# fraunhoferhhi/vvdec

Hardware: NVIDIA H100
Metric: decoded frames/sec, 4K 10-bit Main10 RA, bit-exact YUV vs reference (higher is better)
Workload: dtype int16 samples / int32 accumulate

## Files before the change

vvdec_b200/csrc/k2_inter.cu:

```cuda
#define VVC_TABLE_QUAL static __device__ const __align__(16)
#include "vvc_tables.h"
#include "common.cuh"
#include <algorithm>
#include <cuda.h>

namespace b200 {

constexpr int IFO = 8192;

struct McParams {
  int16_t* dst[3]; int dstStride[3];
  const int16_t* refs[B200_MAX_SLOTS * 3];
  int refStride[3];
  int W, H, bitDepth, ctuSize, chroma;
  int fastOk;
  const b200_pu* pus; const uint32_t* tiles; const int* meta;
  int32_t* dmvrMv;
  const b200_wp* wp;
  const b200_lmcs* lmcs; int lmcsLog2;
  const CUtensorMap* tmaps; uint8_t tmapBuf[B200_MAX_SLOTS];
};

constexpr int TMA_LW = 24, TMA_LH = 23, TMA_CW = 16, TMA_CH = 11;
constexpr int TMA_LWIN = 576, TMA_CWIN = 192;
__device__ __forceinline__ unsigned smem_u32(const void* p) { return (unsigned)__cvta_generic_to_shared(p); }
__device__ __forceinline__ void mbar_init(unsigned long long* bar, int count)
{
  asm volatile("mbarrier.init.shared::cta.b64 [%0], %1;" :: "r"(smem_u32(bar)), "r"(count) : "memory");
  asm volatile("fence.mbarrier_init.release.cluster;" ::: "memory");
}
__device__ __forceinline__ void mbar_expect_tx(unsigned long long* bar, int bytes)
{
  asm volatile("mbarrier.arrive.expect_tx.release.cta.shared::cta.b64 _, [%0], %1;" :: "r"(smem_u32(bar)), "r"(bytes) : "memory");
}
__device__ __forceinline__ void mbar_wait(unsigned long long* bar, int parity)
{
  asm volatile("{\n\t.reg .pred P1;\n\tWAIT_%=:\n\tmbarrier.try_wait.parity.shared::cta.b64 P1, [%0], %1;\n\t@P1 bra DONE_%=;\n\tbra WAIT_%=;\n\tDONE_%=:\n\t}"
               :: "r"(smem_u32(bar)), "r"(parity) : "memory");
}
__device__ __forceinline__ void tma_load_2d(void* smemDst, const CUtensorMap* map, int x, int y, unsigned long long* bar)
{
  asm volatile("cp.async.bulk.tensor.2d.shared::cluster.global.tile.mbarrier::complete_tx::bytes [%0], [%1, {%2, %3}], [%4];"
               :: "r"(smem_u32(smemDst)), "l"(map), "r"(x), "r"(y), "r"(smem_u32(bar)) : "memory");
}

__device__ __forceinline__ void cp_async4(void* smemDst, const void* gmemSrc)
{
  const unsigned d = (unsigned)__cvta_generic_to_shared(smemDst);
  asm volatile("cp.async.ca.shared.global [%0], [%1], 4;\n" :: "r"(d), "l"(gmemSrc));
}
__device__ __forceinline__ void cp_async_wait_all() { asm volatile("cp.async.wait_all;\n" ::: "memory"); }

#define LUMA_OUT(v) (P.lmcs ? lmcs_fwd(P.lmcs, P.lmcsLog2, (v), pmax) : (v))

struct RefPl { const int16_t* p; int w, h, stride; };
__device__ __forceinline__ int ldc(const RefPl& r, int x, int y) { return r.p[(size_t)min(max(y, 0), r.h - 1) * r.stride + min(max(x, 0), r.w - 1)]; }
struct Win { int x0, y0, x1, y1; };
__device__ __forceinline__ int ldw(const RefPl& r, const Win& W, int x, int y) { return ldc(r, min(max(x, W.x0), W.x1), min(max(y, W.y0), W.y1)); }

__device__ __forceinline__ void clip_mv(int& mx, int& my, int x, int y, const McParams& P)
{
  mx = clip3((-P.ctuSize - 8 - x + 1) * 16, (P.W + 8 - x - 1) * 16, mx);
  my = clip3((-P.ctuSize - 8 - y + 1) * 16, (P.H + 8 - y - 1) * 16, my);
}

__device__ __forceinline__ const int8_t* luma_taps(int frac, bool is4x4, bool altHpel)
{
  if (is4x4) return kIfLuma4x4 + frac * 8;
  if (frac == 8 && altHpel) return kIfAltHpel;
  return kIfLuma + frac * 8;
}

__device__ __forceinline__ void load_taps8(const int8_t* t, int f[8])
{
  const int2 w = __ldg(reinterpret_cast<const int2*>(t));
#pragma unroll
  for (int k = 0; k < 4; k++) { f[k] = (w.x << (24 - 8 * k)) >> 24; f[4 + k] = (w.y << (24 - 8 * k)) >> 24; }
}

__device__ __forceinline__ int avg_bi(int p0, int p1, int w1, int hr, int pmax)
{
  int v;
  if (w1 == 4) v = (p0 + p1 + (1 << hr) + 2 * IFO) >> (hr + 1);
  else         v = (p0 * (8 - w1) + p1 * w1 + (1 << (hr + 2)) + (IFO << 3)) >> (hr + 3);
  return clip3(0, pmax, v);
}

__device__ __forceinline__ int wp_uni(const b200_wp* e, int comp, int p, int hr, int pmax)
{
  const int s = e->shift[comp] + hr;
  return clip3(0, pmax, ((e->w0[comp] * (p + IFO) + (s > 0 ? 1 << (s - 1) : 0)) >> s) + e->offset[comp]);
}
__device__ __forceinline__ int wp_bi(const b200_wp* e, int comp, int p0, int p1, int hr, int pmax)
{
  const int s = e->shift[comp] + hr;
  return clip3(0, pmax, (e->w0[comp] * (p0 + IFO) + e->w1[comp] * (p1 + IFO) + ((1 << s) >> 1) + e->offset[comp] * (1 << (s - 1))) >> s);
}

__device__ __forceinline__ int geo_weight(int splitDir, int l2w, int l2h, int x, int y, int sc)
{
  const int angle = kGeoParams[splitDir * 2], mir = kGeoAngle2Mirror[angle];
  const int16_t* wo = &kGeoWeightOffset[((splitDir * 4 + (l2h - 3)) * 4 + (l2w - 3)) * 2];
  const int row = mir == 2 ? VVC_GEO_MASK_SIZE - 1 - wo[1] - (y << sc) : wo[1] + (y << sc);
  const int col = mir == 1 ? VVC_GEO_MASK_SIZE - 1 - wo[0] - (x << sc) : wo[0] + (x << sc);
  return kGeoWeights[(kGeoAngle2Mask[angle] * VVC_GEO_MASK_SIZE + row) * VVC_GEO_MASK_SIZE + col];
}
__device__ __forceinline__ int geo_blend(int wt, int p0, int p1, int hr, int pmax)
{
  const int s = hr + 3;
  return clip3(0, pmax, (wt * p0 + (8 - wt) * p1 + (1 << (s - 1)) + (IFO << 3)) >> s);
}

__device__ __forceinline__ int shift_msb(int numer, int denom) { return numer >> (31 - __clz(denom)); }

__device__ int div_for_maxq7(long long N, long long D)
{
  int sign = 0, q = 0;
  if (N < 0) { sign = 1; N = -N; }
  D <<= 3;
  if (N >= D) { N -= D; q++; }
  q <<= 1; D >>= 1;
  if (N >= D) { N -= D; q++; }
  q <<= 1;
  if (N >= (D >> 1)) q++;
  return sign ? -q : q;
}

struct TileSmem {
  int16_t *w[2], *h[2];
  int16_t *cw[2][2], *chf[2][2];
  int16_t *p[2];
};

constexpr int HS = 16, CHS = 8;
constexpr int DMVR_TAIL = 1640;

__host__ __device__ inline int mc_smem_elems(int mode, int n, bool tma = false)
{
  if (tma) {
    const int lists = mode == 0 ? 1 : 2;
    int e = lists * (TMA_LWIN + 23 * HS + 2 * (TMA_CWIN + 11 * CHS));
    if (mode >= 2) e = max(e, 8 * n) + 2 * 324;
    return (e + 64 + 64) & ~7;
  }
  const int win = n == 256 ? 552 : n == 128 ? 368 : n == 64 ? 276 : 180;
  const int hf  = (n == 256 ? 23 : n == 128 ? 23 : n == 64 ? 23 : 15) * HS;
  const int cwin = n == 256 ? 132 : n == 128 ? 88 : n == 64 ? 66 : 42;
  const int chf = (n == 256 ? 11 : n == 128 ? 11 : n == 64 ? 11 : 7) * CHS;
  const int lists = mode == 0 ? 1 : 2;
  int e = lists * (win + hf + 2 * (cwin + chf));
  if (mode == 3) e = max(e, 2 * 441);
  if (mode >= 2) e = max(e, 8 * n);
  if (mode == 3) e += DMVR_TAIL;
  if (mode >= 2) e += 2 * 324;
  return (e + 64) & ~7;
}

template <int MODE, int OPT, bool TMA>
__device__ __forceinline__ void mc_tile(const McParams& P, const uint32_t tile, int16_t* smem, unsigned* sSad, int* sDec, int (*sVxy)[2], unsigned long long* sBar)
{
  const int tid = threadIdx.x, nthr = blockDim.x;
  const b200_pu& pu = P.pus[tile >> 6];
  const int puW = pu.w, puH = pu.h, puX = pu.x, puY = pu.y, flags = pu.flags;
  const int tx0 = (tile & 7) * 16, ty0 = ((tile >> 3) & 7) * 16;
  const int tw = min(16, puW - tx0), th = min(16, puH - ty0);
  const int l2w = 31 - __clz(tw);
  const int bx = puX + tx0, by = puY + ty0;
  const int bd = P.bitDepth, pmax = (1 << bd) - 1, hr = max(2, 14 - bd), sh1 = 6 - hr;
  constexpr bool BI = MODE != 0;
  const bool altHpel = flags & B200_PU_ALTHPEL;
  const bool is4x4 = puW == 4 && puH == 4;
  const int l0 = BI ? 0 : (pu.refSlot[0] >= 0 ? 0 : 1);
  constexpr int NL = BI ? 2 : 1;
  const int cw = tw >> 1, ch = th >> 1, l2cw = l2w - 1;
  const int chroma = P.chroma;
  const b200_wp* we = (MODE <= 1 && P.wp && pu.wpIdx) ? P.wp + pu.wpIdx - 1 : nullptr;
  const bool geo = MODE == 1 && (flags & B200_PU_GEO);
  const int gl2w = 31 - __clz(puW), gl2h = 31 - __clz(puH);
  const int WS = tw + 8, CS = TMA ? TMA_CW : cw + 4;

  TileSmem S;
  int16_t* tail = smem;
  {
    int16_t* q = smem;
    const int win = WS * (th + 7), hf = (th + 7) * HS, cwin = CS * (ch + 3), chf = (ch + 3) * CHS;
    if (TMA) {
      q += ((128 - (smem_u32(smem) & 127)) & 127) >> 1;
#pragma unroll
      for (int l = 0; l < NL; l++) { S.w[l] = q; q += TMA_LWIN; }
#pragma unroll
      for (int l = 0; l < NL; l++)
#pragma unroll
        for (int c = 0; c < 2; c++) { S.cw[l][c] = q; q += TMA_CWIN; }
#pragma unroll
      for (int l = 0; l < NL; l++) { S.h[l] = q; q += hf; }
#pragma unroll
      for (int l = 0; l < NL; l++)
#pragma unroll
        for (int c = 0; c < 2; c++) { S.chf[l][c] = q; q += chf; }
    } else {
#pragma unroll
    for (int l = 0; l < NL; l++) { S.w[l] = q; q += win; S.h[l] = q; q += hf; }
#pragma unroll
    for (int l = 0; l < NL; l++)
#pragma unroll
      for (int c = 0; c < 2; c++) { S.cw[l][c] = q; q += cwin; S.chf[l][c] = q; q += chf; }
    }
    if (MODE == 3 && q < smem + 2 * 441) q = smem + 2 * 441;
    if (MODE >= 2) { if (q < smem + 8 * tw * th) q = smem + 8 * tw * th; if (MODE == 3) { tail = q; q += DMVR_TAIL; } S.p[0] = q; S.p[1] = q + 324; }
  }

  const int16_t* rp[NL][3]; int mvx[NL], mvy[NL]; int tbuf[NL];
#pragma unroll
  for (int li = 0; li < NL; li++) {
    const int l = BI ? li : l0;
    const int slot = pu.refSlot[l];
    if (TMA) tbuf[li] = P.tmapBuf[slot];
#pragma unroll
    for (int c = 0; c < 3; c++) rp[li][c] = P.refs[slot * 3 + c];
    mvx[li] = pu.mv[l][0]; mvy[li] = pu.mv[l][1];
  }
  const int W = P.W, H = P.H, CWp = W >> 1, CHp = H >> 1, rs0 = P.refStride[0], rs1 = P.refStride[1];
  int ox[NL], oy[NL], ocx[NL], ocy[NL];
  int wx0[NL][2], wy0[NL][2], wx1[NL][2], wy1[NL][2];
  int fmx[NL], fmy[NL];
  bool bio = MODE == 2;

  int wofs[NL], cofs[NL];
  bool dmvrFast = false;
  if (MODE == 3) {
    int16_t* B0 = tail; int16_t* B1 = tail + 400;
    int16_t* B0s = tail + 800; int16_t* B1s = tail + 1200;
    const int BW = tw + 4, BH = th + 4;
    const int warp = tid >> 5, lane = tid & 31, nw = max(1, nthr >> 5);
    int ix[2], iy[2], icx[2], icy[2];
    dmvrFast = P.fastOk;
#pragma unroll
    for (int li = 0; li < 2; li++) {
      ix[li] = bx + (mvx[li] >> 4); iy[li] = by + (mvy[li] >> 4); icx[li] = (bx >> 1) + (mvx[li] >> 5); icy[li] = (by >> 1) + (mvy[li] >> 5);
      dmvrFast = dmvrFast && ix[li] >= 6 && ix[li] + tw + 8 < W && iy[li] >= 6 && iy[li] + th + 8 < H;
      dmvrFast = dmvrFast && (!chroma || (icx[li] >= 4 && icx[li] + cw + 5 < CWp && icy[li] >= 3 && icy[li] + ch + 4 < CHp));
    }
    const int16_t* braw[2]; int bstr;
    int bxF[2], byF[2];
    if (dmvrFast) {
#pragma unroll
      for (int li = 0; li < 2; li++) {
        bxF[li] = mvx[li] & 15; byF[li] = mvy[li] & 15;
        wofs[li] = (ix[li] - 3) & 1;
        {
          const int half = lane >> 4, wl = lane & 15, rw = rs0 >> 1;
          const uint32_t* src = reinterpret_cast<const uint32_t*>(rp[li][0] + (size_t)(iy[li] - 3) * rs0 + ((ix[li] - 3) & ~1)) + (size_t)(warp * 2 + half) * rw + wl;
          uint32_t* dst = reinterpret_cast<uint32_t*>(S.w[li]) + (warp * 2 + half) * (WS >> 1) + wl;
          if (wl < (WS >> 1))
#pragma unroll 4
            for (int y = warp * 2 + half; y < th + 7; y += nw * 2) { cp_async4(dst, src); src += (size_t)(nw * 2) * rw; dst += nw * 2 * (WS >> 1); }
        }
        cofs[li] = (icx[li] - 1) & 1;
        if (chroma) {
          const int sub = lane >> 3, wl = lane & 7, rwc = rs1 >> 1, npc = (ch + 6) >> 2;
          const size_t cbase = (size_t)(icy[li] - 1) * rs1 + ((icx[li] - 1) & ~1);
          for (int q = warp; q < 2 * npc; q += nw) {
// ... 178 lines not shown
      }
    }
#pragma unroll
    for (int li = 0; li < NL; li++) {
      const bool fast = lfast[li];
      wofs[li] = (fast && !TMA) ? ((ox[li] - 3) & 1) : 0;
      if (fast && TMA) {
      } else if (fast) {
        const int half = lane >> 4, wl = lane & 15, rw = rs0 >> 1;
        const uint32_t* src = reinterpret_cast<const uint32_t*>(rp[li][0] + (size_t)(oy[li] - 3) * rs0 + ((ox[li] - 3) & ~1)) + (size_t)(warp * 2 + half) * rw + wl;
        uint32_t* dst = reinterpret_cast<uint32_t*>(S.w[li]) + (warp * 2 + half) * (WS >> 1) + wl;
        if (wl < (WS >> 1))
#pragma unroll 4
          for (int y = warp * 2 + half; y < th + 7; y += nw * 2) { cp_async4(dst, src); src += (size_t)(nw * 2) * rw; dst += nw * 2 * (WS >> 1); }
      } else {
        const int xlo = MODE == 3 ? clip3(0, W - 1, wx0[li][0]) : 0, xhi = MODE == 3 ? clip3(0, W - 1, wx1[li][0]) : W - 1;
        const int ylo = MODE == 3 ? clip3(0, H - 1, wy0[li][0]) : 0, yhi = MODE == 3 ? clip3(0, H - 1, wy1[li][0]) : H - 1;
        const int xc = min(max(ox[li] - 3 + lane, xlo), xhi);
        if (lane < tw + 7)
#pragma unroll 4
          for (int y = warp; y < th + 7; y += nw) S.w[li][y * WS + lane] = __ldg(rp[li][0] + (size_t)min(max(oy[li] - 3 + y, ylo), yhi) * rs0 + xc);
      }
      cofs[li] = 0;
      if (chroma) {
        const bool cfast = cfastv[li];
        cofs[li] = (cfast && !TMA) ? ((ocx[li] - 1) & 1) : 0;
        if (cfast && TMA) {
        } else if (cfast) {
          const int sub = lane >> 3, wl = lane & 7, rwc = rs1 >> 1, npc = (ch + 6) >> 2;
          const size_t cbase = (size_t)(ocy[li] - 1) * rs1 + ((ocx[li] - 1) & ~1);
          for (int q = warp; q < 2 * npc; q += nw) {
            const int c = q >= npc, y = ((c ? q - npc : q) << 2) + sub;
            if (y < ch + 3 && wl < ((cw + 4) >> 1))
              cp_async4(reinterpret_cast<uint32_t*>(c ? S.cw[li][1] : S.cw[li][0]) + y * (CS >> 1) + wl, reinterpret_cast<const uint32_t*>((c ? rp[li][2] : rp[li][1]) + cbase) + (size_t)y * rwc + wl);
          }
        } else {
          const int c = lane >> 4, xl = lane & 15;
          const int xlo = MODE == 3 ? clip3(0, CWp - 1, wx0[li][1]) : 0, xhi = MODE == 3 ? clip3(0, CWp - 1, wx1[li][1]) : CWp - 1;
          const int ylo = MODE == 3 ? clip3(0, CHp - 1, wy0[li][1]) : 0, yhi = MODE == 3 ? clip3(0, CHp - 1, wy1[li][1]) : CHp - 1;
          const int xcc = min(max(ocx[li] - 1 + xl, xlo), xhi);
          const int16_t* rc = c ? rp[li][2] : rp[li][1];
          int16_t* dc = c ? S.cw[li][1] : S.cw[li][0];
          if (xl < cw + 3)
#pragma unroll 4
            for (int y = warp; y < ch + 3; y += nw) dc[y * CS + xl] = __ldg(rc + (size_t)min(max(ocy[li] - 1 + y, ylo), yhi) * rs1 + xcc);
        }
      }
    }
  }
  cp_async_wait_all();
  if (TMA && tmaAny) mbar_wait(sBar, 0);
  __syncthreads();

#pragma unroll
  for (int li = 0; li < NL; li++) {
    int f[8];
    load_taps8(luma_taps(fmx[li] & 15, is4x4, altHpel), f);
    const int16_t* sw = S.w[li] + wofs[li];
    if (OPT == 1) {
      for (int i = tid; i < (th + 7) << l2w; i += nthr) {
        const int y = i >> l2w, x = i & (tw - 1);
        const int16_t* s = sw + y * WS + x;
        int a = 0;
#pragma unroll
        for (int k = 0; k < 8; k++) a += f[k] * s[k];
        S.h[li][y * HS + x] = (int16_t)((a - (IFO << sh1)) >> sh1);
      }
    } else {
      const int l2g = l2w - 2;
      for (int i = tid; i < (th + 7) << l2g; i += nthr) {
        const int y = i >> l2g, x = (i & ((tw >> 2) - 1)) << 2;
        const int16_t* s = sw + y * WS + x;
        int v[11];
#pragma unroll
        for (int k = 0; k < 11; k++) v[k] = s[k];
        int16_t* o = S.h[li] + y * HS + x;
#pragma unroll
        for (int j = 0; j < 4; j++) {
          int a = 0;
#pragma unroll
          for (int k = 0; k < 8; k++) a += f[k] * v[j + k];
          o[j] = (int16_t)((a - (IFO << sh1)) >> sh1);
        }
      }
    }
    if (chroma) {
      const int8_t* t = kIfChroma + (fmx[li] & 31) * 4;
      const int c0 = t[0], c1 = t[1], c2 = t[2], c3 = t[3];
      for (int i = tid; i < 2 * ((ch + 3) << l2cw); i += nthr) {
        const int c = i >= ((ch + 3) << l2cw), j = c ? i - ((ch + 3) << l2cw) : i;
        const int y = j >> l2cw, x = j & (cw - 1);
        const int16_t* s = (c ? S.cw[li][1] : S.cw[li][0]) + cofs[li] + y * CS + x;
        (c ? S.chf[li][1] : S.chf[li][0])[y * CHS + x] = (int16_t)((c0 * s[0] + c1 * s[1] + c2 * s[2] + c3 * s[3] - (IFO << sh1)) >> sh1);
      }
    }
  }
  __syncthreads();

  const int sx = tid & (tw - 1), sy = (tid >> l2w) * OPT;
  {
    int pr[NL][OPT];
#pragma unroll
    for (int li = 0; li < NL; li++) {
      int f[8];
      load_taps8(luma_taps(fmy[li] & 15, is4x4, altHpel), f);
      const int16_t* s = S.h[li] + sy * HS + sx;
      int v[7 + OPT];
#pragma unroll
      for (int k = 0; k < 7 + OPT; k++) v[k] = s[k * HS];
#pragma unroll
      for (int j = 0; j < OPT; j++) {
        int a = 0;
#pragma unroll
        for (int k = 0; k < 8; k++) a += f[k] * v[j + k];
        pr[li][j] = a;
      }
    }
#pragma unroll
    for (int j = 0; j < OPT; j++) {
      int16_t* d = P.dst[0] + (size_t)(by + sy + j) * P.dstStride[0] + bx + sx;
      if (MODE == 1 && geo) *d = (int16_t)LUMA_OUT(geo_blend(geo_weight(pu.bcwW1, gl2w, gl2h, tx0 + sx, ty0 + sy + j, 0), (int16_t)(pr[0][j] >> 6), (int16_t)(pr[NL - 1][j] >> 6), hr, pmax));
      else if (MODE <= 1 && we) *d = (int16_t)LUMA_OUT(BI ? wp_bi(we, 0, (int16_t)(pr[0][j] >> 6), (int16_t)(pr[NL - 1][j] >> 6), hr, pmax) : wp_uni(we, 0, (int16_t)(pr[0][j] >> 6), hr, pmax));
      else if (!BI) *d = (int16_t)LUMA_OUT(clip3(0, pmax, (pr[0][j] + (1 << (5 + hr)) + (IFO << 6)) >> (6 + hr)));
      else if (!bio) *d = (int16_t)LUMA_OUT(avg_bi((int16_t)(pr[0][j] >> 6), (int16_t)(pr[NL - 1][j] >> 6), MODE == 1 ? pu.bcwW1 : 4, hr, pmax));
      else { S.p[0][(sy + j + 1) * 18 + sx + 1] = (int16_t)(pr[0][j] >> 6); S.p[1][(sy + j + 1) * 18 + sx + 1] = (int16_t)(pr[NL - 1][j] >> 6); }
    }
  }
  if (chroma) {
    for (int i = tid; i < 2 * (ch << l2cw); i += nthr) {
      const int c = i >= (ch << l2cw), j = c ? i - (ch << l2cw) : i;
      const int y = j >> l2cw, x = j & (cw - 1);
      int pr[NL];
#pragma unroll
      for (int li = 0; li < NL; li++) {
        const int8_t* t = kIfChroma + (fmy[li] & 31) * 4;
        const int16_t* s = (c ? S.chf[li][1] : S.chf[li][0]) + y * CHS + x;
        pr[li] = t[0] * s[0] + t[1] * s[CHS] + t[2] * s[2 * CHS] + t[3] * s[3 * CHS];
      }
      int16_t* d = (c ? P.dst[2] : P.dst[1]) + (size_t)((by >> 1) + y) * (c ? P.dstStride[2] : P.dstStride[1]) + (bx >> 1) + x;
      if (MODE == 1 && geo) *d = (int16_t)geo_blend(geo_weight(pu.bcwW1, gl2w, gl2h, (tx0 >> 1) + x, (ty0 >> 1) + y, 1), (int16_t)(pr[0] >> 6), (int16_t)(pr[NL - 1] >> 6), hr, pmax);
      else if (MODE <= 1 && we) *d = (int16_t)(BI ? wp_bi(we, 1 + c, (int16_t)(pr[0] >> 6), (int16_t)(pr[NL - 1] >> 6), hr, pmax) : wp_uni(we, 1 + c, (int16_t)(pr[0] >> 6), hr, pmax));
      else if (!BI) *d = (int16_t)clip3(0, pmax, (pr[0] + (1 << (5 + hr)) + (IFO << 6)) >> (6 + hr));
      else *d = (int16_t)avg_bi((int16_t)(pr[0] >> 6), (int16_t)(pr[NL - 1] >> 6), MODE == 1 ? pu.bcwW1 : 4, hr, pmax);
    }
  }

  if (MODE >= 2) {
    if (!bio) return;
    for (int i = tid; i < 4 * (tw + th + 2); i += nthr) {
      const int li = i >= 2 * (tw + th + 2), j = li ? i - 2 * (tw + th + 2) : i;
      int x, y;
      if (j < tw + 2) { x = j; y = 0; } else if (j < 2 * (tw + 2)) { x = j - (tw + 2); y = th + 1; }
      else if (j < 2 * (tw + 2) + th) { x = 0; y = j - 2 * (tw + 2) + 1; } else { x = tw + 1; y = j - 2 * (tw + 2) - th + 1; }
      const int mxl = li ? fmx[NL - 1] : fmx[0], myl = li ? fmy[NL - 1] : fmy[0];
      const int xo = (mxl & 15) < 8 ? 1 : 0, yo = (myl & 15) < 8 ? 1 : 0;
      const int16_t* wl = li ? S.w[NL - 1] + wofs[NL - 1] : S.w[0] + wofs[0];
      const int v = wl[(y - yo + 3) * WS + (x - xo + 3)];
      (li ? S.p[1] : S.p[0])[y * 18 + x] = (int16_t)((int16_t)(v << hr) - IFO);
    }
    __syncthreads();
    uint4* Q = reinterpret_cast<uint4*>(smem);
    int dgx[OPT], dgy[OPT], psum[OPT];
    {
      int q0[OPT + 2], q1[OPT + 2];
#pragma unroll
      for (int r = 0; r < OPT + 2; r++) { q0[r] = S.p[0][(sy + r) * 18 + sx + 1] >> 6; q1[r] = S.p[1][(sy + r) * 18 + sx + 1] >> 6; }
#pragma unroll
      for (int j = 0; j < OPT; j++) {
        const int i = (sy + j + 1) * 18 + sx + 1;
        const int p0 = S.p[0][i], p1 = S.p[1][i];
        const int g0x = (S.p[0][i + 1] >> 6) - (S.p[0][i - 1] >> 6), g1x = (S.p[1][i + 1] >> 6) - (S.p[1][i - 1] >> 6);
        const int g0y = q0[j + 2] - q0[j], g1y = q1[j + 2] - q1[j];
        const int tX = (g0x + g1x) >> 1, tY = (g0y + g1y) >> 1, dI = (p1 >> 4) - (p0 >> 4);
        uint4 rec;
        rec.x = (unsigned)abs(tX) | ((unsigned)abs(tY) << 16);
        rec.y = (unsigned)(tX < 0 ? -dI : (tX == 0 ? 0 : dI));
        rec.z = (unsigned)(tY < 0 ? -dI : (tY == 0 ? 0 : dI));
        rec.w = (unsigned)(tY < 0 ? -tX : (tY == 0 ? 0 : tX));
        Q[((sy + j) << l2w) + sx] = rec;
        dgx[j] = g0x - g1x; dgy[j] = g0y - g1y; psum[j] = p0 + p1;
      }
    }
    __syncthreads();
    const int nBlk = (tw >> 2) * (th >> 2), l2bw = l2w - 2;
    for (int it = tid; it < ((nBlk * 4 + 31) & ~31); it += nthr) {
      const int blk = it >> 2, part = it & 3;
      unsigned sA = 0; int sDX = 0, sDY = 0, sS = 0;
      if (blk < nBlk) {
        const int bxx = (blk & ((tw >> 2) - 1)) << 2, byy = (blk >> l2bw) << 2;
#pragma unroll
        for (int rr = 0; rr < 2; rr++) {
          const int yy = part + 4 * rr;
          if (yy < 6) {
            const uint4* row = Q + (min(max(byy + yy - 1, 0), th - 1) << l2w);
#pragma unroll
            for (int xx = 0; xx < 6; xx++) {
              const uint4 r = row[min(max(bxx + xx - 1, 0), tw - 1)];
              sA += r.x; sDX += (int)r.y; sDY += (int)r.z; sS += (int)r.w;
            }
          }
        }
      }
#pragma unroll
      for (int m = 1; m < 4; m <<= 1) {
        sA += __shfl_xor_sync(0xffffffffu, sA, m);
        sDX += __shfl_xor_sync(0xffffffffu, sDX, m); sDY += __shfl_xor_sync(0xffffffffu, sDY, m);
        sS  += __shfl_xor_sync(0xffffffffu, sS, m);
      }
      if (part == 0 && blk < nBlk) {
        const int sAX = sA & 0xffff, sAY = sA >> 16;
        int vx = sAX == 0 ? 0 : shift_msb(sDX * 4, sAX);
        vx = clip3(-15, 15, vx);
        const int mainG = sS >> 12, secG = sS & 4095;
        int tmp = vx * mainG;
        tmp = ((tmp * (1 << 12)) + vx * secG) >> 1;
        int vy = sAY == 0 ? 0 : shift_msb(sDY * 4 - tmp, sAY);
        vy = clip3(-15, 15, vy);
        sVxy[blk][0] = vx; sVxy[blk][1] = vy;
      }
    }
    __syncthreads();
#pragma unroll
    for (int j = 0; j < OPT; j++) {
      const int y = sy + j, blk = ((y >> 2) << l2bw) + (sx >> 2);
      const int b = sVxy[blk][0] * dgx[j] + sVxy[blk][1] * dgy[j];
      const int shiftNum = 15 - bd, offset = (1 << (shiftNum - 1)) + 2 * IFO;
      P.dst[0][(size_t)(by + y) * P.dstStride[0] + bx + sx] = (int16_t)LUMA_OUT(clip3(0, pmax, (int)(int16_t)((psum[j] + b + offset) >> shiftNum)));
    }
  }
}

template <int MODE, int OPT, bool TMA>
__global__ void __launch_bounds__(64, MODE >= 2 ? 12 : 16) mc_kernel(const McParams P, const int list)
{
  extern __shared__ __align__(128) int16_t smem[];
  __shared__ unsigned sSad[25];
  __shared__ int sDec[3];
  __shared__ int sVxy[16][2];
  __shared__ __align__(8) unsigned long long sBar;
  if ((int)blockIdx.x >= P.meta[LM_CNT + list]) return;
  if (TMA) { if (threadIdx.x == 0) mbar_init(&sBar, 1); __syncthreads(); }
  mc_tile<MODE, OPT, TMA>(P, P.tiles[P.meta[LM_OFF + list] + blockIdx.x], smem, sSad, sDec, sVxy, &sBar);
}

__device__ __forceinline__ void round_affine(int& x, int& y, int s) { const int o = 1 << (s - 1); x = (x + o - (x >= 0)) >> s; y = (y + o - (y >= 0)) >> s; }

__device__ bool spread_over_limit(int a, int b, int c, int d, int predType)
{
  const int s4 = 4 << 11, ft = 6;
  if (predType == 3) {
    int rw = max(max(0, 4 * a + s4), max(4 * c, 4 * a + 4 * c + s4)) - min(min(0, 4 * a + s4), min(4 * c, 4 * a + 4 * c + s4));
    int rh = max(max(0, 4 * b), max(4 * d + s4, 4 * b + 4 * d + s4)) - min(min(0, 4 * b), min(4 * d + s4, 4 * b + 4 * d + s4));
    rw = (rw >> 11) + ft + 3; rh = (rh >> 11) + ft + 3;
    return rw * rh > (ft + 9) * (ft + 9);
  }
  int rw = max(0, 4 * a + s4) - min(0, 4 * a + s4), rh = max(0, 4 * b) - min(0, 4 * b);
  rw = (rw >> 11) + ft + 3; rh = (rh >> 11) + ft + 3;
  if (rw * rh > (ft + 9) * (ft + 5)) return true;
  rw = max(0, 4 * c) - min(0, 4 * c); rh = max(0, 4 * d + s4) - min(0, 4 * d + s4);
  rw = (rw >> 11) + ft + 3; rh = (rh >> 11) + ft + 3;
  return rw * rh > (ft + 5) * (ft + 9);
}

struct AffModel { int LTx, LTy, dHX, dHY, dVX, dVY; bool over, prof; };

__device__ void aff_model(const b200_pu& pu, int l, AffModel& M)
{
  const int l2w = 31 - __clz((int)pu.w), l2h = 31 - __clz((int)pu.h);
  M.LTx = pu.mv[l][0]; M.LTy = pu.mv[l][1];
  const int RTx = pu.cpmv[l][0][0], RTy = pu.cpmv[l][0][1], LBx = pu.cpmv[l][1][0], LBy = pu.cpmv[l][1][1];
  const bool six = pu.flags & B200_PU_AFFINE6;
  M.dHX = (RTx - M.LTx) * (1 << (7 - l2w)); M.dHY = (RTy - M.LTy) * (1 << (7 - l2w));
  M.dVX = six ? (LBx - M.LTx) * (1 << (7 - l2h)) : -M.dHY; M.dVY = six ? (LBy - M.LTy) * (1 << (7 - l2h)) : M.dHX;
  M.over = spread_over_limit(M.dHX, M.dHY, M.dVX, M.dVY, pu.interDir);
  bool prof = pu.flags & (l ? B200_PU_PROF1 : B200_PU_PROF0);
  if (six ? (M.LTx == RTx && M.LTy == RTy && M.LTx == LBx && M.LTy == LBy) : (M.LTx == RTx && M.LTy == RTy)) prof = false;
  if (M.over) prof = false;
  M.prof = prof;
}

__device__ __forceinline__ void aff_sub_mv(const AffModel& M, const b200_pu& pu, int i, int j, int& mx, int& my)
{
  if (M.over) { mx = M.LTx * 128 + M.dHX * (pu.w >> 1) + M.dVX * (pu.h >> 1); my = M.LTy * 128 + M.dHY * (pu.w >> 1) + M.dVY * (pu.h >> 1); }
  else        { mx = M.LTx * 128 + M.dHX * (2 + 4 * i) + M.dVX * (2 + 4 * j); my = M.LTy * 128 + M.dHY * (2 + 4 * i) + M.dVY * (2 + 4 * j); }
  round_affine(mx, my, 7);
  mx = clip3(-(1 << 17), (1 << 17) - 1, mx); my = clip3(-(1 << 17), (1 << 17) - 1, my);
}

__device__ __forceinline__ void mc_affine_tile(const McParams& P, const uint32_t tile)
{
  __shared__ int16_t sHf[2][16][9 * 4];
  __shared__ int16_t sE[2][16][36];
  __shared__ int16_t sP[2][3][256];
  __shared__ int16_t sCH[2][2][4][7 * 4];

// ... 88 lines not shown
      const int i0 = (tx0 >> 2) + (csx >> 1), j0 = (ty0 >> 2) + (csy >> 1);
      aff_sub_mv(Ml, pu, i0, j0, ax, ay); aff_sub_mv(Ml, pu, i0 + 1, j0 + 1, bxm, bym);
      mx = ax + bxm; my = ay + bym;
      round_affine(mx, my, 1);
      mx = clip3(hMin, hMax, mx); my = clip3(vMin, vMax, my);
    }
    const int xF = mx & 31, yF = my & 31, X0 = (bx >> 1) + csx + (mx >> 5), Y0 = (by >> 1) + csy + (my >> 5);
    if (valid) {
      const int8_t* fh = kIfChroma + xF * 4;
      for (int j = k; j < 28; j += 16) {
        const int y = j >> 2, x = j & 3;
        int s = 0;
#pragma unroll
        for (int t = 0; t < 4; t++) s += fh[t] * ldc(Rc, X0 + x + t - 1, Y0 + y - 1);
        sCH[li][c - 1][cs][j] = (int16_t)((s - (IFO << sh1)) >> sh1);
      }
    }
    __syncwarp();
    if (valid) {
      const int y = k >> 2, x = k & 3;
      const int8_t* fv = kIfChroma + yF * 4;
      int s = 0;
#pragma unroll
      for (int t = 0; t < 4; t++) s += fv[t] * sCH[li][c - 1][cs][(y + t) * 4 + x];
      if (bi) sP[l][c][(csy + y) * 8 + csx + x] = (int16_t)(s >> 6);
      else P.dst[c][(size_t)((by >> 1) + csy + y) * P.dstStride[c] + (bx >> 1) + csx + x] = (int16_t)(we ? wp_uni(we, c, (int16_t)(s >> 6), hr, pmax) : clip3(0, pmax, (s + (1 << (5 + hr)) + (IFO << 6)) >> (6 + hr)));
    }
  }
  if (!bi) return;
  __syncthreads();
  {
    const int y = tid >> 4, x = tid & 15;
    if (x < tw && y < th) P.dst[0][(size_t)(by + y) * P.dstStride[0] + bx + x] = (int16_t)LUMA_OUT(we ? wp_bi(we, 0, sP[0][0][y * 16 + x], sP[1][0][y * 16 + x], hr, pmax) : avg_bi(sP[0][0][y * 16 + x], sP[1][0][y * 16 + x], pu.bcwW1, hr, pmax));
    if (P.chroma && tid < 128) {
      const int c = tid >> 6, j = tid & 63, yy = j >> 3, xx = j & 7;
      if (xx < (tw >> 1) && yy < (th >> 1))
        P.dst[1 + c][(size_t)((by >> 1) + yy) * P.dstStride[1 + c] + (bx >> 1) + xx] = (int16_t)(we ? wp_bi(we, 1 + c, sP[0][1 + c][yy * 8 + xx], sP[1][1 + c][yy * 8 + xx], hr, pmax) : avg_bi(sP[0][1 + c][yy * 8 + xx], sP[1][1 + c][yy * 8 + xx], pu.bcwW1, hr, pmax));
    }
  }
}

__global__ void __launch_bounds__(256) mc_affine_kernel(const McParams P)
{
  if ((int)blockIdx.x >= P.meta[LM_CNT + 16]) return;
  mc_affine_tile(P, P.tiles[P.meta[LM_OFF + 16] + blockIdx.x]);
}

int launch_mc(const McLaunch& L, StreamSet& ss, KProf* prof)
{
  McParams P;
  for (int c = 0; c < 3; c++) { P.dst[c] = L.dst.p[c]; P.dstStride[c] = L.dst.stride[c]; P.refStride[c] = L.refStride[c]; }
  for (int i = 0; i < B200_MAX_SLOTS * 3; i++) P.refs[i] = L.refs[i];
  P.fastOk = !(L.refStride[0] & 1) && !(L.refStride[1] & 1) && !(L.refStride[2] & 1);
  P.W = L.geom.width; P.H = L.geom.height; P.bitDepth = L.geom.bitDepth; P.ctuSize = L.geom.ctuSize; P.chroma = L.geom.chromaFormat == 1;
  P.pus = L.pus; P.dmvrMv = L.dmvrMv; P.tiles = L.tiles; P.meta = L.meta;
  P.wp = L.wp;
  P.lmcs = L.lmcs; P.lmcsLog2 = 0; { int o = (1 << L.geom.bitDepth) / 16; while ((1 << (P.lmcsLog2 + 1)) <= o) P.lmcsLog2++; }
  P.tmaps = reinterpret_cast<const CUtensorMap*>(L.tmaps); memcpy(P.tmapBuf, L.tmapBuf, sizeof(P.tmapBuf));
  static const bool tmaEnv = getenv("B200_MC_TMA") && !strcmp(getenv("B200_MC_TMA"), "1");
  const bool tmaOn = P.tmaps && P.chroma && tmaEnv;
  int launched = 0;
  if (prof) prof->begin(B200_KF_MC_TILE, ss.main);
  for (int m = 3; m >= 0; m--) for (int k = 3; k >= 0; k--) {
    const int nsamp = 32 << k, list = m * 4 + k, grid = L.cnt[list];
    if (!grid || (m >= 2 && k < 2)) continue;
    cudaStream_t s = ss.pick(launched++);
    const bool tma = tmaOn && k == 3 && m <= 2;
    const size_t smem = (size_t)mc_smem_elems(m, nsamp, tma) * 2;
    if (tma) {
      switch (m) {
        case 0: mc_kernel<0, 4, true><<<grid, 64, smem, s>>>(P, list); break;
        case 1: mc_kernel<1, 4, true><<<grid, 64, smem, s>>>(P, list); break;
        default: mc_kernel<2, 4, true><<<grid, 64, smem, s>>>(P, list); break;
      }
    } else if (k >= 2) {
      const int nthr = nsamp >> 2;
      switch (m) {
        case 0: mc_kernel<0, 4, false><<<grid, nthr, smem, s>>>(P, list); break;
        case 1: mc_kernel<1, 4, false><<<grid, nthr, smem, s>>>(P, list); break;
        case 2: mc_kernel<2, 4, false><<<grid, nthr, smem, s>>>(P, list); break;
        default: mc_kernel<3, 4, false><<<grid, nthr, smem, s>>>(P, list); break;
      }
    } else {
      switch (m) {
        case 0: mc_kernel<0, 1, false><<<grid, nsamp, smem, s>>>(P, list); break;
        default: mc_kernel<1, 1, false><<<grid, nsamp, smem, s>>>(P, list); break;
      }
    }
    B200_CUDA(cudaGetLastError());
  }
  if (L.cnt[16]) { cudaStream_t s = ss.pick(launched++); mc_affine_kernel<<<L.cnt[16], 256, 0, s>>>(P); B200_CUDA(cudaGetLastError()); }
  ss.join();
  if (prof) prof->end(B200_KF_MC_TILE, ss.main);
  return 0;
}

int make_mc_tensor_maps(const b200_geom& g, int16_t* const* bufPlanes, int nBufs, void** out)
{
  *out = nullptr;
  if (g.chromaFormat != 1 || (g.stride[0] & 7) || (g.stride[1] & 7) || (g.stride[2] & 7)) return 0;
  typedef CUresult (*EncodeFn)(CUtensorMap*, CUtensorMapDataType, cuuint32_t, void*, const cuuint64_t*, const cuuint64_t*, const cuuint32_t*, const cuuint32_t*,
                               CUtensorMapInterleave, CUtensorMapSwizzle, CUtensorMapL2promotion, CUtensorMapFloatOOBfill);
  void* fn = nullptr; cudaDriverEntryPointQueryResult qres;
  if (cudaGetDriverEntryPoint("cuTensorMapEncodeTiled", &fn, cudaEnableDefault, &qres) != cudaSuccess || qres != cudaDriverEntryPointSuccess || !fn) { cudaGetLastError(); return 0; }
  std::vector<CUtensorMap> maps((size_t)nBufs * 3);
  for (int i = 0; i < nBufs * 3; i++) {
    const int c = i % 3;
    if ((uintptr_t)bufPlanes[i] & 15) return 0;
    const cuuint64_t dims[2] = {(cuuint64_t)(c ? g.width >> 1 : g.width), (cuuint64_t)(c ? g.height >> 1 : g.height)};
    const cuuint64_t strides[1] = {(cuuint64_t)g.stride[c] * 2};
    const cuuint32_t box[2] = {(cuuint32_t)(c ? TMA_CW : TMA_LW), (cuuint32_t)(c ? TMA_CH : TMA_LH)}, estr[2] = {1, 1};
    const CUresult r = reinterpret_cast<EncodeFn>(fn)(&maps[i], CU_TENSOR_MAP_DATA_TYPE_UINT16, 2, bufPlanes[i], dims, strides, box, estr, CU_TENSOR_MAP_INTERLEAVE_NONE,
                                                     CU_TENSOR_MAP_SWIZZLE_NONE, CU_TENSOR_MAP_L2_PROMOTION_NONE, CU_TENSOR_MAP_FLOAT_OOB_FILL_NONE);
    if (r != CUDA_SUCCESS) return 0;
  }
  B200_CUDA(cudaMalloc(out, maps.size() * sizeof(CUtensorMap)));
  B200_CUDA(cudaMemcpy(*out, maps.data(), maps.size() * sizeof(CUtensorMap), cudaMemcpyHostToDevice));
  return 0;
}

int mc_launch_count(const McLaunch& L) { int n = L.cnt[16] > 0; for (int m = 0; m < 4; m++) for (int k = 0; k < 4; k++) n += L.cnt[m * 4 + k] > 0 && !(m >= 2 && k < 2); return n; }

}
```

Baseline: 1138.

## Vectorize MC separable filter with dp2a on packed int16 pairs and even/odd row planes

Result: no change. 1128, median of 6 (-0.9%).

```diff
diff --git a/vvdec_b200/csrc/k2_inter.cu b/vvdec_b200/csrc/k2_inter.cu
--- a/vvdec_b200/csrc/k2_inter.cu
+++ b/vvdec_b200/csrc/k2_inter.cu
@@ -14,6 +14,7 @@
   int refStride[3];
   int W, H, bitDepth, ctuSize, chroma;
   int fastOk;
+  int vecOk;
   const b200_pu* pus; const uint32_t* tiles; const int* meta;
   int32_t* dmvrMv;
   const b200_wp* wp;
@@ -69,13 +70,6 @@
   if (is4x4) return kIfLuma4x4 + frac * 8;
   if (frac == 8 && altHpel) return kIfAltHpel;
   return kIfLuma + frac * 8;
-}
-
-__device__ __forceinline__ void load_taps8(const int8_t* t, int f[8])
-{
-  const int2 w = __ldg(reinterpret_cast<const int2*>(t));
-#pragma unroll
-  for (int k = 0; k < 4; k++) { f[k] = (w.x << (24 - 8 * k)) >> 24; f[4 + k] = (w.y << (24 - 8 * k)) >> 24; }
 }
 
 __device__ __forceinline__ int avg_bi(int p0, int p1, int w1, int hr, int pmax)
@@ -127,34 +121,59 @@
 }
 
 struct TileSmem {
-  int16_t *w[2], *h[2];
-  int16_t *cw[2][2], *chf[2][2];
+  int16_t *w[2];
+  uint32_t *pe[2], *po[2];
+  int16_t *cw[2][2];
+  uint32_t *cpe[2][2], *cpo[2][2];
   int16_t *p[2];
 };
 
 constexpr int HS = 16, CHS = 8;
 constexpr int DMVR_TAIL = 1640;
 
+struct TileLayout { int w[2], pe[2], po[2], cw[2][2], cpe[2][2], cpo[2][2], tail, p, end; };
+__host__ __device__ inline int al8(int n) { return (n + 7) & ~7; }
+__host__ __device__ inline TileLayout mc_layout(int mode, int tw, int th, bool tma)
+{
+  TileLayout L = {};
+  const int nl = mode == 0 ? 1 : 2, cw = tw >> 1, ch = th >> 1;
+  const int win = tma ? TMA_LWIN : al8((tw + 8) * (th + 7)), cwin = tma ? TMA_CWIN : al8((cw + 4) * (ch + 3));
+  const int hf = ((th >> 1) + 4) * HS * 2, chf = ((ch >> 1) + 2) * CHS * 2;
+  int q = 0;
+  for (int l = 0; l < nl; l++) { L.w[l] = q; q += win; }
+  for (int l = 0; l < nl; l++) for (int c = 0; c < 2; c++) { L.cw[l][c] = q; q += cwin; }
+  for (int l = 0; l < nl; l++) { L.pe[l] = q; q += hf; L.po[l] = q; q += hf; }
+  for (int l = 0; l < nl; l++) for (int c = 0; c < 2; c++) { L.cpe[l][c] = q; q += chf; L.cpo[l][c] = q; q += chf; }
+  if (mode == 3) q = max(q, 2 * 441);
+  if (mode >= 2) q = max(q, 8 * tw * th);
+  if (mode == 3) { L.tail = q; q += DMVR_TAIL; }
+  if (mode >= 2) { L.p = q; q += 2 * 324; }
+  L.end = al8(q);
+  return L;
+}
+
 __host__ __device__ inline int mc_smem_elems(int mode, int n, bool tma = false)
 {
-  if (tma) {
-    const int lists = mode == 0 ? 1 : 2;
-    int e = lists * (TMA_LWIN + 23 * HS + 2 * (TMA_CWIN + 11 * CHS));
-    if (mode >= 2) e = max(e, 8 * n) + 2 * 324;
-    return (e + 64 + 64) & ~7;
-  }
-  const int win = n == 256 ? 552 : n == 128 ? 368 : n == 64 ? 276 : 180;
-  const int hf  = (n == 256 ? 23 : n == 128 ? 23 : n == 64 ? 23 : 15) * HS;
-  const int cwin = n == 256 ? 132 : n == 128 ? 88 : n == 64 ? 66 : 42;
-  const int chf = (n == 256 ? 11 : n == 128 ? 11 : n == 64 ? 11 : 7) * CHS;
-  const int lists = mode == 0 ? 1 : 2;
-  int e = lists * (win + hf + 2 * (cwin + chf));
-  if (mode == 3) e = max(e, 2 * 441);
-  if (mode >= 2) e = max(e, 8 * n);
-  if (mode == 3) e += DMVR_TAIL;
-  if (mode >= 2) e += 2 * 324;
-  return (e + 64) & ~7;
-}
+  if (tma) return mc_layout(mode, 16, 16, true).end + 64;
+  int e = 0;
+  for (int tw = 4; tw <= 16; tw <<= 1)
+    if (n / tw >= 4 && n / tw <= 16) e = max(e, mc_layout(mode, tw, n / tw, false).end);
+  return e;
+}
+
+template <int N>
+__device__ __forceinline__ void pair_words(const uint32_t (&w)[N + 1], bool odd, uint32_t (&e)[N], uint32_t (&o)[N])
+{
+#pragma unroll
+  for (int k = 0; k < N; k++) { const uint32_t m = __byte_perm(w[k], w[k + 1], 0x5432); e[k] = odd ? m : w[k]; o[k] = odd ? w[k + 1] : m; }
+}
+__device__ __forceinline__ int dot8(uint32_t a, uint32_t b, uint32_t c, uint32_t d, int t0, int t1)
+{
+  return __dp2a_hi((int)d, t1, __dp2a_lo((int)c, t1, __dp2a_hi((int)b, t0, __dp2a_lo((int)a, t0, 0))));
+}
+__device__ __forceinline__ int dot4(uint32_t a, uint32_t b, int t) { return __dp2a_hi((int)b, t, __dp2a_lo((int)a, t, 0)); }
+__device__ __forceinline__ void st_half(uint32_t* a, int i, int hi, int v) { reinterpret_cast<int16_t*>(a + i)[hi] = (int16_t)v; }
+__device__ __forceinline__ uint32_t pk2(int a, int b) { return __byte_perm(a, b, 0x5410); }
 
 template <int MODE, int OPT, bool TMA>
 __device__ __forceinline__ void mc_tile(const McParams& P, const uint32_t tile, int16_t* smem, unsigned* sSad, int* sDec, int (*sVxy)[2], unsigned long long* sBar)
@@ -180,34 +199,20 @@
   const int WS = tw + 8, CS = TMA ? TMA_CW : cw + 4;
 
   TileSmem S;
-  int16_t* tail = smem;
+  int16_t* tail;
   {
-    int16_t* q = smem;
-    const int win = WS * (th + 7), hf = (th + 7) * HS, cwin = CS * (ch + 3), chf = (ch + 3) * CHS;
-    if (TMA) {
-      q += ((128 - (smem_u32(smem) & 127)) & 127) >> 1;
-#pragma unroll
-      for (int l = 0; l < NL; l++) { S.w[l] = q; q += TMA_LWIN; }
-#pragma unroll
-      for (int l = 0; l < NL; l++)
-#pragma unroll
-        for (int c = 0; c < 2; c++) { S.cw[l][c] = q; q += TMA_CWIN; }
-#pragma unroll
-      for (int l = 0; l < NL; l++) { S.h[l] = q; q += hf; }
-#pragma unroll
-      for (int l = 0; l < NL; l++)
-#pragma unroll
-        for (int c = 0; c < 2; c++) { S.chf[l][c] = q; q += chf; }
-    } else {
-#pragma unroll
-    for (int l = 0; l < NL; l++) { S.w[l] = q; q += win; S.h[l] = q; q += hf; }
-#pragma unroll
-    for (int l = 0; l < NL; l++)
-#pragma unroll
-      for (int c = 0; c < 2; c++) { S.cw[l][c] = q; q += cwin; S.chf[l][c] = q; q += chf; }
-    }
-    if (MODE == 3 && q < smem + 2 * 441) q = smem + 2 * 441;
-    if (MODE >= 2) { if (q < smem + 8 * tw * th) q = smem + 8 * tw * th; if (MODE == 3) { tail = q; q += DMVR_TAIL; } S.p[0] = q; S.p[1] = q + 324; }
+    int16_t* b = smem;
+    if (TMA) b += ((128 - (smem_u32(smem) & 127)) & 127) >> 1;
+    const TileLayout L = mc_layout(MODE, tw, th, TMA);
+#pragma unroll
+    for (int l = 0; l < NL; l++) {
+      S.w[l] = b + L.w[l]; S.pe[l] = reinterpret_cast<uint32_t*>(b + L.pe[l]); S.po[l] = reinterpret_cast<uint32_t*>(b + L.po[l]);
+#pragma unroll
+      for (int c = 0; c < 2; c++) {
+        S.cw[l][c] = b + L.cw[l][c]; S.cpe[l][c] = reinterpret_cast<uint32_t*>(b + L.cpe[l][c]); S.cpo[l][c] = reinterpret_cast<uint32_t*>(b + L.cpo[l][c]);
+      }
+    }
+    tail = b + L.tail; S.p[0] = b + L.p; S.p[1] = b + L.p + 324;
   }
 
   const int16_t* rp[NL][3]; int mvx[NL], mvy[NL]; int tbuf[NL];
@@ -492,98 +497,117 @@
   if (TMA && tmaAny) mbar_wait(sBar, 0);
   __syncthreads();
 
+  const int l2g = l2w - 2, l2cg = l2cw - 1;
 #pragma unroll
   for (int li = 0; li < NL; li++) {
-    int f[8];
-    load_taps8(luma_taps(fmx[li] & 15, is4x4, altHpel), f);
-    const int16_t* sw = S.w[li] + wofs[li];
-    if (OPT == 1) {
-      for (int i = tid; i < (th + 7) << l2w; i += nthr) {
-        const int y = i >> l2w, x = i & (tw - 1);
-        const int16_t* s = sw + y * WS + x;
-        int a = 0;
-#pragma unroll
-        for (int k = 0; k < 8; k++) a += f[k] * s[k];
-        S.h[li][y * HS + x] = (int16_t)((a - (IFO << sh1)) >> sh1);
-      }
-    } else {
-      const int l2g = l2w - 2;
-      for (int i = tid; i < (th + 7) << l2g; i += nthr) {
-        const int y = i >> l2g, x = (i & ((tw >> 2) - 1)) << 2;
-        const int16_t* s = sw + y * WS + x;
-        int v[11];
-#pragma unroll
-        for (int k = 0; k < 11; k++) v[k] = s[k];
-        int16_t* o = S.h[li] + y * HS + x;
-#pragma unroll
-        for (int j = 0; j < 4; j++) {
-          int a = 0;
-#pragma unroll
-          for (int k = 0; k < 8; k++) a += f[k] * v[j + k];
-          o[j] = (int16_t)((a - (IFO << sh1)) >> sh1);
-        }
+    const int2 t = __ldg(reinterpret_cast<const int2*>(luma_taps(fmx[li] & 15, is4x4, altHpel)));
+    const bool odd = wofs[li];
+    const uint32_t* sw = reinterpret_cast<const uint32_t*>(S.w[li]);
+    for (int i = tid; i < (th + 7) << l2g; i += nthr) {
+      const int y = i >> l2g, x = (i & ((tw >> 2) - 1)) << 2;
+      const uint32_t* s = sw + ((y * WS + x) >> 1);
+      uint32_t w[6], e[5], o[5];
+#pragma unroll
+      for (int k = 0; k < 6; k++) w[k] = s[k];
+      pair_words<5>(w, odd, e, o);
+#pragma unroll
+      for (int j = 0; j < 4; j++) {
+        const uint32_t* p = (j & 1) ? o + (j >> 1) : e + (j >> 1);
+        const int v = (dot8(p[0], p[1], p[2], p[3], t.x, t.y) - (IFO << sh1)) >> sh1;
+        st_half(S.pe[li], (y >> 1) * HS + x + j, y & 1, v);
+        if (y) st_half(S.po[li], ((y - 1) >> 1) * HS + x + j, (y - 1) & 1, v);
       }
     }
     if (chroma) {
-      const int8_t* t = kIfChroma + (fmx[li] & 31) * 4;
-      const int c0 = t[0], c1 = t[1], c2 = t[2], c3 = t[3];
-      for (int i = tid; i < 2 * ((ch + 3) << l2cw); i += nthr) {
-        const int c = i >= ((ch + 3) << l2cw), j = c ? i - ((ch + 3) << l2cw) : i;
-        const int y = j >> l2cw, x = j & (cw - 1);
-        const int16_t* s = (c ? S.cw[li][1] : S.cw[li][0]) + cofs[li] + y * CS + x;
-        (c ? S.chf[li][1] : S.chf[li][0])[y * CHS + x] = (int16_t)((c0 * s[0] + c1 * s[1] + c2 * s[2] + c3 * s[3] - (IFO << sh1)) >> sh1);
+      const int t4 = __ldg(reinterpret_cast<const int*>(kIfChroma + (fmx[li] & 31) * 4));
+      const bool codd = cofs[li];
+      const int n = (ch + 3) << l2cg;
+      for (int i = tid; i < 2 * n; i += nthr) {
+        const int c = i >= n, j = c ? i - n : i;
+        const int y = j >> l2cg, x = (j & ((cw >> 1) - 1)) << 1;
+        const uint32_t* s = reinterpret_cast<const uint32_t*>(c ? S.cw[li][1] : S.cw[li][0]) + ((y * CS + x) >> 1);
+        uint32_t w[3], e[2], o[2];
+#pragma unroll
+        for (int k = 0; k < 3; k++) w[k] = s[k];
+        pair_words<2>(w, codd, e, o);
+        uint32_t* pe = c ? S.cpe[li][1] : S.cpe[li][0];
+        uint32_t* po = c ? S.cpo[li][1] : S.cpo[li][0];
+#pragma unroll
+        for (int k = 0; k < 2; k++) {
+          const int v = (dot4(k ? o[0] : e[0], k ? o[1] : e[1], t4) - (IFO << sh1)) >> sh1;
+          st_half(pe, (y >> 1) * CHS + x + k, y & 1, v);
+          if (y) st_half(po, ((y - 1) >> 1) * CHS + x + k, (y - 1) & 1, v);
+        }
       }
     }
   }
   __syncthreads();
 
+  {
+    int2 tv[NL];
+#pragma unroll
+    for (int li = 0; li < NL; li++) tv[li] = __ldg(reinterpret_cast<const int2*>(luma_taps(fmy[li] & 15, is4x4, altHpel)));
+    for (int i = tid; i < th << l2g; i += nthr) {
+      const int y = i >> l2g, x = (i & ((tw >> 2) - 1)) << 2;
+      int pr[NL][4];
+#pragma unroll
+      for (int li = 0; li < NL; li++) {
+        const uint4* s = reinterpret_cast<const uint4*>(((y & 1) ? S.po[li] : S.pe[li]) + (y >> 1) * HS + x);
+        uint4 r[4];
+#pragma unroll
+        for (int k = 0; k < 4; k++) r[k] = s[k * (HS / 4)];
+        pr[li][0] = dot8(r[0].x, r[1].x, r[2].x, r[3].x, tv[li].x, tv[li].y);
+        pr[li][1] = dot8(r[0].y, r[1].y, r[2].y, r[3].y, tv[li].x, tv[li].y);
+        pr[li][2] = dot8(r[0].z, r[1].z, r[2].z, r[3].z, tv[li].x, tv[li].y);
+        pr[li][3] = dot8(r[0].w, r[1].w, r[2].w, r[3].w, tv[li].x, tv[li].y);
+      }
+      if (MODE >= 2 && bio) {
+#pragma unroll
+        for (int j = 0; j < 4; j++) { S.p[0][(y + 1) * 18 + x + j + 1] = (int16_t)(pr[0][j] >> 6); S.p[1][(y + 1) * 18 + x + j + 1] = (int16_t)(pr[NL - 1][j] >> 6); }
+        continue;
+      }
+      int v[4];
+#pragma unroll
+      for (int j = 0; j < 4; j++) {
+        if (MODE == 1 && geo) v[j] = LUMA_OUT(geo_blend(geo_weight(pu.bcwW1, gl2w, gl2h, tx0 + x + j, ty0 + y, 0), (int16_t)(pr[0][j] >> 6), (int16_t)(pr[NL - 1][j] >> 6), hr, pmax));
+        else if (MODE <= 1 && we) v[j] = LUMA_OUT(BI ? wp_bi(we, 0, (int16_t)(pr[0][j] >> 6), (int16_t)(pr[NL - 1][j] >> 6), hr, pmax) : wp_uni(we, 0, (int16_t)(pr[0][j] >> 6), hr, pmax));
+        else if (!BI) v[j] = LUMA_OUT(clip3(0, pmax, (pr[0][j] + (1 << (5 + hr)) + (IFO << 6)) >> (6 + hr)));
+        else v[j] = LUMA_OUT(avg_bi((int16_t)(pr[0][j] >> 6), (int16_t)(pr[NL - 1][j] >> 6), MODE == 1 ? pu.bcwW1 : 4, hr, pmax));
+      }
+      int16_t* d = P.dst[0] + (size_t)(by + y) * P.dstStride[0] + bx + x;
+      if (P.vecOk) *reinterpret_cast<uint2*>(d) = make_uint2(pk2(v[0], v[1]), pk2(v[2], v[3]));
+      else { d[0] = (int16_t)v[0]; d[1] = (int16_t)v[1]; d[2] = (int16_t)v[2]; d[3] = (int16_t)v[3]; }
+    }
+  }
+  if (chroma) {
+    int tc[NL];
+#pragma unroll
+    for (int li = 0; li < NL; li++) tc[li] = __ldg(reinterpret_cast<const int*>(kIfChroma + (fmy[li] & 31) * 4));
+    const int n = ch << l2cg;
+    for (int i = tid; i < 2 * n; i += nthr) {
+      const int c = i >= n, j = c ? i - n : i;
+      const int y = j >> l2cg, x = (j & ((cw >> 1) - 1)) << 1;
+      int pr[NL][2];
+#pragma unroll
+      for (int li = 0; li < NL; li++) {
+        const uint2* s = reinterpret_cast<const uint2*>(((y & 1) ? (c ? S.cpo[li][1] : S.cpo[li][0]) : (c ? S.cpe[li][1] : S.cpe[li][0])) + (y >> 1) * CHS + x);
+        const uint2 r0 = s[0], r1 = s[CHS / 2];
+        pr[li][0] = dot4(r0.x, r1.x, tc[li]); pr[li][1] = dot4(r0.y, r1.y, tc[li]);
+      }
+      int v[2];
+#pragma unroll
+      for (int k = 0; k < 2; k++) {
+        if (MODE == 1 && geo) v[k] = geo_blend(geo_weight(pu.bcwW1, gl2w, gl2h, (tx0 >> 1) + x + k, (ty0 >> 1) + y, 1), (int16_t)(pr[0][k] >> 6), (int16_t)(pr[NL - 1][k] >> 6), hr, pmax);
+        else if (MODE <= 1 && we) v[k] = BI ? wp_bi(we, 1 + c, (int16_t)(pr[0][k] >> 6), (int16_t)(pr[NL - 1][k] >> 6), hr, pmax) : wp_uni(we, 1 + c, (int16_t)(pr[0][k] >> 6), hr, pmax);
+        else if (!BI) v[k] = clip3(0, pmax, (pr[0][k] + (1 << (5 + hr)) + (IFO << 6)) >> (6 + hr));
+        else v[k] = avg_bi((int16_t)(pr[0][k] >> 6), (int16_t)(pr[NL - 1][k] >> 6), MODE == 1 ? pu.bcwW1 : 4, hr, pmax);
+      }
+      int16_t* d = (c ? P.dst[2] : P.dst[1]) + (size_t)((by >> 1) + y) * (c ? P.dstStride[2] : P.dstStride[1]) + (bx >> 1) + x;
+      if (P.vecOk) *reinterpret_cast<uint32_t*>(d) = pk2(v[0], v[1]);
+      else { d[0] = (int16_t)v[0]; d[1] = (int16_t)v[1]; }
+    }
+  }
   const int sx = tid & (tw - 1), sy = (tid >> l2w) * OPT;
-  {
-    int pr[NL][OPT];
-#pragma unroll
-    for (int li = 0; li < NL; li++) {
-      int f[8];
-      load_taps8(luma_taps(fmy[li] & 15, is4x4, altHpel), f);
-      const int16_t* s = S.h[li] + sy * HS + sx;
-      int v[7 + OPT];
-#pragma unroll
-      for (int k = 0; k < 7 + OPT; k++) v[k] = s[k * HS];
-#pragma unroll
-      for (int j = 0; j < OPT; j++) {
-        int a = 0;
-#pragma unroll
-        for (int k = 0; k < 8; k++) a += f[k] * v[j + k];
-        pr[li][j] = a;
-      }
-    }
-#pragma unroll
-    for (int j = 0; j < OPT; j++) {
-      int16_t* d = P.dst[0] + (size_t)(by + sy + j) * P.dstStride[0] + bx + sx;
-      if (MODE == 1 && geo) *d = (int16_t)LUMA_OUT(geo_blend(geo_weight(pu.bcwW1, gl2w, gl2h, tx0 + sx, ty0 + sy + j, 0), (int16_t)(pr[0][j] >> 6), (int16_t)(pr[NL - 1][j] >> 6), hr, pmax));
-      else if (MODE <= 1 && we) *d = (int16_t)LUMA_OUT(BI ? wp_bi(we, 0, (int16_t)(pr[0][j] >> 6), (int16_t)(pr[NL - 1][j] >> 6), hr, pmax) : wp_uni(we, 0, (int16_t)(pr[0][j] >> 6), hr, pmax));
-      else if (!BI) *d = (int16_t)LUMA_OUT(clip3(0, pmax, (pr[0][j] + (1 << (5 + hr)) + (IFO << 6)) >> (6 + hr)));
-      else if (!bio) *d = (int16_t)LUMA_OUT(avg_bi((int16_t)(pr[0][j] >> 6), (int16_t)(pr[NL - 1][j] >> 6), MODE == 1 ? pu.bcwW1 : 4, hr, pmax));
-      else { S.p[0][(sy + j + 1) * 18 + sx + 1] = (int16_t)(pr[0][j] >> 6); S.p[1][(sy + j + 1) * 18 + sx + 1] = (int16_t)(pr[NL - 1][j] >> 6); }
-    }
-  }
-  if (chroma) {
-    for (int i = tid; i < 2 * (ch << l2cw); i += nthr) {
-      const int c = i >= (ch << l2cw), j = c ? i - (ch << l2cw) : i;
-      const int y = j >> l2cw, x = j & (cw - 1);
-      int pr[NL];
-#pragma unroll
-      for (int li = 0; li < NL; li++) {
-        const int8_t* t = kIfChroma + (fmy[li] & 31) * 4;
-        const int16_t* s = (c ? S.chf[li][1] : S.chf[li][0]) + y * CHS + x;
-        pr[li] = t[0] * s[0] + t[1] * s[CHS] + t[2] * s[2 * CHS] + t[3] * s[3 * CHS];
-      }
-      int16_t* d = (c ? P.dst[2] : P.dst[1]) + (size_t)((by >> 1) + y) * (c ? P.dstStride[2] : P.dstStride[1]) + (bx >> 1) + x;
-      if (MODE == 1 && geo) *d = (int16_t)geo_blend(geo_weight(pu.bcwW1, gl2w, gl2h, (tx0 >> 1) + x, (ty0 >> 1) + y, 1), (int16_t)(pr[0] >> 6), (int16_t)(pr[NL - 1] >> 6), hr, pmax);
-      else if (MODE <= 1 && we) *d = (int16_t)(BI ? wp_bi(we, 1 + c, (int16_t)(pr[0] >> 6), (int16_t)(pr[NL - 1] >> 6), hr, pmax) : wp_uni(we, 1 + c, (int16_t)(pr[0] >> 6), hr, pmax));
-      else if (!BI) *d = (int16_t)clip3(0, pmax, (pr[0] + (1 << (5 + hr)) + (IFO << 6)) >> (6 + hr));
-      else *d = (int16_t)avg_bi((int16_t)(pr[0] >> 6), (int16_t)(pr[NL - 1] >> 6), MODE == 1 ? pu.bcwW1 : 4, hr, pmax);
-    }
-  }
 
   if (MODE >= 2) {
     if (!bio) return;
@@ -671,16 +695,17 @@
 }
 
 template <int MODE, int OPT, bool TMA>
-__global__ void __launch_bounds__(64, MODE >= 2 ? 12 : 16) mc_kernel(const McParams P, const int list)
+__global__ void __launch_bounds__(64, MODE >= 2 ? 14 : 24) mc_kernel(const McParams P, const int list)
 {
   extern __shared__ __align__(128) int16_t smem[];
   __shared__ unsigned sSad[25];
   __shared__ int sDec[3];
   __shared__ int sVxy[16][2];
   __shared__ __align__(8) unsigned long long sBar;
-  if ((int)blockIdx.x >= P.meta[LM_CNT + list]) return;
+  const int cnt = P.meta[LM_CNT + list], off = P.meta[LM_OFF + list];
+  if ((int)blockIdx.x >= cnt) return;
   if (TMA) { if (threadIdx.x == 0) mbar_init(&sBar, 1); __syncthreads(); }
-  mc_tile<MODE, OPT, TMA>(P, P.tiles[P.meta[LM_OFF + list] + blockIdx.x], smem, sSad, sDec, sVxy, &sBar);
+  mc_tile<MODE, OPT, TMA>(P, P.tiles[off + blockIdx.x], smem, sSad, sDec, sVxy, &sBar);
 }
 
 __device__ __forceinline__ void round_affine(int& x, int& y, int s) { const int o = 1 << (s - 1); x = (x + o - (x >= 0)) >> s; y = (y + o - (y >= 0)) >> s; }
@@ -875,6 +900,7 @@
   for (int c = 0; c < 3; c++) { P.dst[c] = L.dst.p[c]; P.dstStride[c] = L.dst.stride[c]; P.refStride[c] = L.refStride[c]; }
   for (int i = 0; i < B200_MAX_SLOTS * 3; i++) P.refs[i] = L.refs[i];
   P.fastOk = !(L.refStride[0] & 1) && !(L.refStride[1] & 1) && !(L.refStride[2] & 1);
+  P.vecOk = !((uintptr_t)L.dst.p[0] & 7) && !(L.dst.stride[0] & 3) && !((uintptr_t)L.dst.p[1] & 3) && !(L.dst.stride[1] & 1) && !((uintptr_t)L.dst.p[2] & 3) && !(L.dst.stride[2] & 1);
   P.W = L.geom.width; P.H = L.geom.height; P.bitDepth = L.geom.bitDepth; P.ctuSize = L.geom.ctuSize; P.chroma = L.geom.chromaFormat == 1;
   P.pus = L.pus; P.dmvrMv = L.dmvrMv; P.tiles = L.tiles; P.meta = L.meta;
   P.wp = L.wp;
@@ -882,12 +908,14 @@
   P.tmaps = reinterpret_cast<const CUtensorMap*>(L.tmaps); memcpy(P.tmapBuf, L.tmapBuf, sizeof(P.tmapBuf));
   static const bool tmaEnv = getenv("B200_MC_TMA") && !strcmp(getenv("B200_MC_TMA"), "1");
   const bool tmaOn = P.tmaps && P.chroma && tmaEnv;
+  const char* serialEnv = getenv("B200_MC_SERIAL");
+  const bool serial = serialEnv && !strcmp(serialEnv, "1");
   int launched = 0;
   if (prof) prof->begin(B200_KF_MC_TILE, ss.main);
   for (int m = 3; m >= 0; m--) for (int k = 3; k >= 0; k--) {
     const int nsamp = 32 << k, list = m * 4 + k, grid = L.cnt[list];
     if (!grid || (m >= 2 && k < 2)) continue;
-    cudaStream_t s = ss.pick(launched++);
+    cudaStream_t s = serial ? ss.main : ss.pick(launched++);
     const bool tma = tmaOn && k == 3 && m <= 2;
     const size_t smem = (size_t)mc_smem_elems(m, nsamp, tma) * 2;
     if (tma) {
@@ -912,7 +940,7 @@
     }
     B200_CUDA(cudaGetLastError());
   }
-  if (L.cnt[16]) { cudaStream_t s = ss.pick(launched++); mc_affine_kernel<<<L.cnt[16], 256, 0, s>>>(P); B200_CUDA(cudaGetLastError()); }
+  if (L.cnt[16]) { cudaStream_t s = serial ? ss.main : ss.pick(launched++); mc_affine_kernel<<<L.cnt[16], 256, 0, s>>>(P); B200_CUDA(cudaGetLastError()); }
   ss.join();
   if (prof) prof->end(B200_KF_MC_TILE, ss.main);
   return 0;
```
